# WestlyPark/StyleRenderer

Measured on AMD Instinct MI355X. Metric: generator fwd+bwd images/sec at 256^2, higher is better.
Workload: dtype f32

## Files before the change

### include/stylerenderer_amd.h

```cpp
#ifndef STYLERENDERER_AMD_H_
#define STYLERENDERER_AMD_H_

#include <stddef.h>
#include <stdint.h>

#ifdef __cplusplus
extern "C" {
#endif

typedef void* sr_stream_t;

#define SR_OK 0
#define SR_EINVAL (-1)
#define SR_ERANGE (-2)

const char* sr_error_string(int code);
int sr_abi_version(void);

int sr_fused_bias_act(float* y, const float* x, const float* b, const float* ref, int act, int grad,
                      float alpha, float scale, int64_t size_x, int64_t step_b, int64_t size_b,
                      int use_bias, int use_ref, sr_stream_t stream);

int64_t sr_fused_act_bwd_scratch_floats(int64_t n, int64_t c, int64_t inner);
int sr_fused_act_bwd(float* gx, float* gb, const float* gy, const float* out, float alpha,
// ... 34 lines not shown
int sr_adam_flat_guarded(float* p, const float* g, float* m, float* v, int64_t n, float lr, float beta1, float beta2,
                         float eps, float* step, const int64_t* guard_offs, int n_guards,
                         int32_t* skipped_host, sr_stream_t stream);

int64_t sr_rowdot_scratch_floats(int64_t rows, int64_t inner);
int sr_rowdot(float* dots, float* out_scaled, const float* a, const float* b, const float* scale,
              int64_t rows, int64_t inner, float* scratch, sr_stream_t stream);
int sr_rowdot_div(float* dots, const float* a, const float* b, const float* rdiv, int64_t rows, int64_t inner,
                  float* scratch, sr_stream_t stream);
int sr_rowdot_bwd(float* ga, float* gb, float* gs, const float* a, const float* b, const float* gd, const float* go,
                  const float* scale, int64_t rows, int64_t inner, float* scratch, sr_stream_t stream);

int sr_smallconv_fwd(float* out, const float* x, const float* ws, const float* bias, int64_t B, int64_t C,
                     int64_t N, int64_t hw, sr_stream_t stream);
int sr_smallconv_dx(float* dx, const float* g, const float* ws, int64_t B, int64_t C, int64_t N, int64_t hw,
                    sr_stream_t stream);
int sr_smallconv_dx_add(float* dx, const float* g, const float* ws, const float* addend, int64_t B, int64_t C, int64_t N,
                        int64_t hw, sr_stream_t stream);
int64_t sr_smallconv_dw_scratch_floats(int64_t B, int64_t C, int64_t N, int64_t hw);
int sr_smallconv_dw(float* dws, const float* g, const float* x, int64_t B, int64_t C, int64_t N, int64_t hw,
                    float* scratch, sr_stream_t stream);
int sr_smallconv_dw_bias(float* dws, float* gb, const float* g, const float* x, int64_t B, int64_t C, int64_t N, int64_t hw,
                         float* scratch, sr_stream_t stream);
int sr_modrows_fwd(float* ws, const float* w, const float* s, float scale, int64_t B, int64_t N, int64_t C,
                   sr_stream_t stream);
int sr_modrows_bwd(float* gs, float* gw, const float* dws, const float* w, const float* s, float scale, int64_t B,
                   int64_t N, int64_t C, sr_stream_t stream);

int sr_vertex_normals_f32(float* vn, float* norm_out, const float* v, const int64_t* tri, const int32_t* adj_off,
                          const int32_t* adj, int64_t B, int64_t nv, int64_t nf, float eps, sr_stream_t stream);

int sr_affine3_fwd(float* out, const float* v, const float* m, const float* t, int64_t B, int64_t nv,
                   int64_t v_bstride, sr_stream_t stream);
int sr_affine3_bwd(float* gm, float* gt, const float* v, const float* g, int64_t B, int64_t nv, int64_t v_bstride,
                   sr_stream_t stream);

int sr_morph_fwd(float* v, float* vs, float* reg, const float* w, const float* bias, const float* coeff, const float* lin,
                 const float* pose, const float* sigma, float lam, int64_t B, int64_t nv, int64_t d, sr_stream_t stream);
int sr_vertex_normals_bwd_f32(float* gvs, const float* gv, const float* gn, const float* lin, const float* rot,
                              const float* v, const float* ns, const float* normc, const int64_t* tri,
                              const int32_t* adj_off, const int32_t* adj, int64_t B, int64_t nv, int64_t nf, float eps,
                              sr_stream_t stream);
int64_t sr_morph_gcoeff_scratch_floats(int64_t rows, int64_t B, int64_t d);
int sr_morph_gcoeff(float* gcoeff, float* scratch, const float* w, const float* gvs, const float* coeff,
                    const float* sigma, float lam, const float* greg, int64_t B, int64_t rows, int64_t d,
                    sr_stream_t stream);
// ... 350 lines not shown
```

### stylerenderer_amd/_lib.py

```python
import ctypes
import os

_HERE = os.path.dirname(os.path.abspath(__file__))
LIB_PATH = os.environ.get("STYLERENDERER_AMD_LIB") or os.path.join(_HERE, "libstylerenderer_hip.so")

_i = ctypes.c_int
_l = ctypes.c_int64
_f = ctypes.c_float
_d = ctypes.c_double
_p = ctypes.c_void_p

SIGNATURES = {
    "sr_error_string": (ctypes.c_char_p, [_i]),
    "sr_abi_version": (_i, []),
    "sr_fused_bias_act": (_i, [_p, _p, _p, _p, _i, _i, _f, _f, _l, _l, _l, _i, _i, _p]),
    "sr_fused_act_bwd_scratch_floats": (_l, [_l, _l, _l]),
    "sr_fused_act_bwd": (_i, [_p, _p, _p, _p, _f, _f, _l, _l, _l, _p, _p]),
    "sr_noise_bias_act": (_i, [_p] * 6 + [_f, _f] + [_l] * 4 + [_p]),
    "sr_noise_bias_act_bwd_scratch_floats": (_l, [_l, _l, _l]),
    "sr_noise_bias_act_bwd": (_i, [_p] * 6 + [_f, _f] + [_l] * 4 + [_p, _p]),
    "sr_noise_bias_act_bwd_dot_scratch_floats": (_l, [_l, _l, _l]),
    "sr_noise_bias_act_bwd_dot": (_i, [_p] * 9 + [_f, _f] + [_l] * 4 + [_p, _p]),
    "sr_conv2d_nba": (_i, [_p] * 8 + [_f, _f] + [_l] * 7 + [_p, _p]),
    "sr_conv2d_nba_ex": (_i, [_p] * 8 + [_f, _f] + [_l] * 7 + [_i, _p, _p]),
    "sr_noise_bias_act_affine": (_i, [_p] * 4 + [_l] + [_p] * 3 + [_f, _f] + [_l] * 4 + [_p]),
    "sr_noise_bias_act_affine_bwd_scratch_floats": (_l, [_l, _l, _l]),
    "sr_noise_bias_act_affine_bwd": (_i, [_p] * 9 + [_l, _p, _f, _f] + [_l] * 4 + [_p, _p]),
    "sr_noise_bias_act_affine_bwd2_scratch_floats": (_l, [_l, _l, _l]),
    "sr_noise_bias_act_affine_bwd2": (_i, [_p, _p, _p, _l, _p, _p, _l] + [_p] * 6 + [_l, _p, _f, _f] + [_l] * 4 + [_p, _p]),
    "sr_adam_flat": (_i, [_p] * 4 + [_l] + [_f] * 4 + [_p, _p]),
    "sr_adam_flat_guarded": (_i, [_p] * 4 + [_l] + [_f] * 4 + [_p, ctypes.POINTER(_l), _i, _p, _p]),
    "sr_rowdot_scratch_floats": (_l, [_l, _l]),
    "sr_rowdot": (_i, [_p] * 5 + [_l, _l, _p, _p]),
    "sr_rowdot_div": (_i, [_p] * 4 + [_l, _l, _p, _p]),
    "sr_rowdot_bwd": (_i, [_p] * 8 + [_l, _l, _p, _p]),
    "sr_smallconv_fwd": (_i, [_p] * 4 + [_l] * 4 + [_p]),
    "sr_smallconv_dx": (_i, [_p] * 3 + [_l] * 4 + [_p]),
    "sr_smallconv_dx_add": (_i, [_p] * 4 + [_l] * 4 + [_p]),
    "sr_smallconv_dw_scratch_floats": (_l, [_l] * 4),
    "sr_smallconv_dw": (_i, [_p] * 3 + [_l] * 4 + [_p, _p]),
    "sr_smallconv_dw_bias": (_i, [_p] * 4 + [_l] * 4 + [_p, _p]),
    "sr_modrows_fwd": (_i, [_p] * 3 + [_f] + [_l] * 3 + [_p]),
    "sr_modrows_bwd": (_i, [_p] * 5 + [_f] + [_l] * 3 + [_p]),
    "sr_vertex_normals_f32": (_i, [_p] * 6 + [_l] * 3 + [_f, _p]),
    "sr_linear_fwd": (_i, [_p] * 4 + [_l] * 4 + [_f, _f, _i, _f, _f, _p]),
    "sr_linear_bwd_x": (_i, [_p] * 4 + [_l] * 3 + [_f, _i, _f, _f, _p]),
    "sr_linear_bwd_w": (_i, [_p] * 5 + [_l] * 4 + [_f, _f, _i, _f, _f, _p]),
    "sr_demod_fwd": (_i, [_p] * 3 + [_l] * 3 + [_f, _p]),
    "sr_demod_bwd": (_i, [_p] * 7 + [_l] * 3 + [_p]),
    "sr_weight_prep": (_i, [_p, _p, _p, _f, _l, _l, _i, _l, _p]),
    "sr_weight_prep_bwd": (_i, [_p, _p, _p, _p, _f, _l, _l, _i, _l, _p]),
    "sr_weight_adjoint": (_i, [_p, _p, _l, _l, _l, _l, _l, _i, _p]),
    "sr_bank_nt": (_i, [_i] + [_p] * 8 + [_l, _f, _f, _p]),
    "sr_bank_nn": (_i, [_i] + [_p] * 8 + [_l, _f, _p]),
    "sr_bank_tn": (_i, [_i] + [_p] * 8 + [_l, _f, _f, _p]),
    "sr_weight_prep_batch": (_i, [_i] + [_p] * 9),
    "sr_weight_adjoint_batch": (_i, [_i] + [_p] * 9),
    "sr_lpips_layer_scratch_floats": (_l, [_l, _l]),
    "sr_lpips_layer_fwd": (_i, [_p] * 4 + [_l] * 4 + [_f, _p, _p]),
    "sr_lpips_layer_bwd": (_i, [_p] * 5 + [_l] * 4 + [_f, _p]),
    "sr_ppl_endpoints": (_i, [_p, _p, _p, _l, _p, _l, _l, _i, _i, _f, _p]),
    "sr_ppl_prep": (_i, [_p] * 4 + [_l] * 9 + [_p]),
    "sr_lpips_pair_scratch_floats": (_l, [_l, _l, _p]),
    "sr_lpips_pair": (_i, [_p] * 5 + [_l, _l, _f, _p, _p]),
# ... 162 lines not shown
```

### stylerenderer_amd/csrc/fused_elem.hip

```cpp
#include "common.h"

namespace {

constexpr int EB = 256;
constexpr int ECHUNK = EB * 16;

__device__ __forceinline__ void block_sum2(float& a, float& b, float* lds8) {
    a = sr_wave_sum(a);
    b = sr_wave_sum(b);
    const int lane = threadIdx.x & 63, wave = threadIdx.x >> 6;
    if (lane == 0) { lds8[wave] = a; lds8[4 + wave] = b; }
    __syncthreads();
    if (threadIdx.x == 0) {
        a = (lds8[0] + lds8[1]) + (lds8[2] + lds8[3]);
        b = (lds8[4] + lds8[5]) + (lds8[6] + lds8[7]);
    }
}

template <bool REF>
__global__ __launch_bounds__(EB) void k_nba_fwd(float* __restrict__ y, const float* __restrict__ x,
                                                const float* __restrict__ noise,
                                                const float* __restrict__ noise_w,
                                                const float* __restrict__ bias,
                                                const float* __restrict__ ref, float alpha, float scale,
// ... 952 lines not shown
        const dim3 grid((unsigned)chunks, (unsigned)(B * C));
        switch (N) {
            case 1: hipLaunchKernelGGL((k_smallconv_dw<1, 1>), grid, dim3(256), 0, st, scratch, g, x, (int)C, hw, chunks, direct, gsum); break;
            case 2: hipLaunchKernelGGL((k_smallconv_dw<2, 1>), grid, dim3(256), 0, st, scratch, g, x, (int)C, hw, chunks, direct, gsum); break;
            case 3: hipLaunchKernelGGL((k_smallconv_dw<3, 1>), grid, dim3(256), 0, st, scratch, g, x, (int)C, hw, chunks, direct, gsum); break;
            default: hipLaunchKernelGGL((k_smallconv_dw<4, 1>), grid, dim3(256), 0, st, scratch, g, x, (int)C, hw, chunks, direct, gsum); break;
        }
    }
    if (chunks > 1)
        hipLaunchKernelGGL(k_smallconv_dw_finish, dim3((unsigned)(B * C)), dim3(64), 0, st, dws, scratch, (int)C,
                           (int)N, chunks, B * C);
    if (gb)
        hipLaunchKernelGGL(k_smallconv_gb_finish, dim3(1), dim3(64), 0, st, gb, gsum, (int)N, (int)(B * chunks));
    return sr_launch_status();
}

extern "C" int sr_smallconv_dw(float* dws, const float* g, const float* x, int64_t B, int64_t C, int64_t N,
                               int64_t hw, float* scratch, sr_stream_t stream) {
    return sr_smallconv_dw_bias(dws, nullptr, g, x, B, C, N, hw, scratch, stream);
}

namespace {

__global__ __launch_bounds__(256) void k_modrows_fwd(float* __restrict__ ws, const float* __restrict__ w,
                                                     const float* __restrict__ s, float scale, int B, int N, int C) {
    const int64_t i = (int64_t)blockIdx.x * 256 + threadIdx.x;
    if (i >= (int64_t)B * N * C) return;
    const int c = (int)(i % C);
    const int j = (int)((i / C) % N);
    const int b = (int)(i / ((int64_t)C * N));
    ws[i] = (w[(int64_t)j * C + c] * scale) * s[(int64_t)b * C + c];
}

__global__ __launch_bounds__(256) void k_modrows_bwd(float* __restrict__ gs, float* __restrict__ gw,
                                                     const float* __restrict__ dws, const float* __restrict__ w,
                                                     const float* __restrict__ s, float scale, int B, int N, int C) {
    const int c = blockIdx.x * 256 + threadIdx.x;
    if (c >= C) return;
    const int r = blockIdx.y;
    if (r < B) {
        if (!gs) return;
        float acc = 0.0f;
        for (int j = 0; j < N; ++j) acc += dws[((int64_t)r * N + j) * C + c] * (w[(int64_t)j * C + c] * scale);
        gs[(int64_t)r * C + c] = acc;
    } else {
        if (!gw) return;
// ... 122 lines not shown
```

### stylerenderer_amd/layers.py

```python
import math
import os

import torch
from torch import nn
from torch.nn import functional as F

from .op import FusedLeakyReLU, fused_leaky_relu, upfirdn2d
from .op import conv as _conv
from .op import conv_generic as _convg
from .op import smallconv as _smallconv
from .op import style as _style
from .op.style_bank import StylePack
from .op.upfirdn2d import skip_down as _skip_down
from .op.weight_prep import weight_prep as _weight_prep
from .op.weight_prep import weight_prep_cached as _weight_prep_cached
from .op._dispatch import strict_native as _strict_native


def _fused_tails():
    import os

    return os.environ.get("SR_FUSED_TAILS", "1") != "0"


def make_kernel(k):
    k = torch.tensor(k, dtype=torch.float32)
    if k.dim() == 1:
        k = k[None, :] * k[:, None]
    return k / k.sum()


class PixelNorm(nn.Module):
# ... 219 lines not shown
            return _conv.conv2d(input, wt, s, d, None, "c3")
        return _conv.conv2d(input, wt, s, d, None, "c1")

    def _forward_generic(self, input, s, skip_blur=False):
        w = self.weight[0] * self.scale
        x = input * s[:, :, None, None]
        d = None
        if self.demodulate:
            wsq = w.pow(2).sum((2, 3)).t().contiguous()
            if _style.demod_supported(s, wsq):
                d = _style.demod_scale(s, wsq, self.eps)
            else:
                d = torch.rsqrt(((s * s)[:, :, None] * wsq[None]).sum(1) + self.eps)
        if self.upsample:
            out = _convg.conv_transpose2d_generic(x, w.transpose(0, 1), stride=2, padding=0)
        elif self.downsample:
            out = _convg.conv2d_generic(self.blur(x), w, None, 2, 0)
        else:
            out = _convg.conv2d_generic(x, w, None, 1, self.padding)
        if d is not None:
            out = out * d[:, :, None, None]
        return self.blur(out) if (self.upsample and not skip_blur) else out

    def forward_noise_bias_act(self, input, style, noise, noise_weight, act_bias, negative_slope, act_scale):
        if (input.device.type != "cuda" or self.upsample or self.downsample or self.kernel_size != 3
                or not self.demodulate or act_bias is None or not _fused_tails()):
            return None
        input = input.contiguous()
        if not _conv.conv_nba_shape_ok(input, self.out_channel, noise):
            return None
        s = self.style_of(style)
        if isinstance(style, StylePack) and style.d is not None:
            wt, wsq, d = style.wt, style.wsq, style.d
            if not _conv.conv_nba_supported(input, wt, noise):
                return None
        else:
            wt, wsq = self._wprep(True)
            if not (_conv.conv_nba_supported(input, wt, noise) and _style.demod_supported(s, wsq)):
                return None
            d = _style.demod_scale(s, wsq, self.eps)
        return _conv.conv2d_nba(input, wt, s, d, noise, noise_weight, act_bias, negative_slope, act_scale)

    def forward_up_noise_bias_act(self, input, style, noise, noise_weight, act_bias, negative_slope, act_scale):
        if (input.device.type != "cuda" or not self.upsample or self.kernel_size != 3 or not self.demodulate
                or act_bias is None or not _fused_tails()):
            return None
        s = self.style_of(style)
        pad = self.blur.pad
        oh = 2 * input.shape[2] + 1 + pad[0] + pad[1] - 3
        ow = 2 * input.shape[3] + 1 + pad[0] + pad[1] - 3
        if isinstance(style, StylePack) and style.d is not None:
            wt, wsq, d = style.wt, style.wsq, style.d
            if not _conv.upconv_nba_supported(input, wt, noise, oh, ow):
                return None
        else:
            wt, wsq = self._wprep(True)
            if not (_conv.upconv_nba_supported(input, wt, noise, oh, ow) and _style.demod_supported(s, wsq)):
                return None
            d = _style.demod_scale(s, wsq, self.eps)
        kernel = self.blur.kernel
        return _conv.upconv_nba(input.contiguous(), wt, s, d, kernel, pad, noise, noise_weight, act_bias,
                                negative_slope, act_scale)

# ... 202 lines not shown
```

### stylerenderer_amd/model.py

```python
import math

import numpy as np
import torch
from torch import nn

from .layers import (BiasBank, Blur, ConstantInput, ConvLayer, EqualLinear, ModulatedConv2d, NoiseInjection,
                     PixelNorm, ResBlock, Upsample)
from .op import FusedLeakyReLU, rasterize
from .op import smallconv as _smallconv
from .op import style_bank as _style_bank
from .op import weight_bank as _weight_bank
from .op.fused_elem import blur_noise_bias_act, noise_bias_act, noise_bias_act_affine
from .op.rasterize import rasterize_pyramid
from .op.upfirdn2d import upsample2_add

CHANNEL_BASE = {4: 512, 8: 512, 16: 512, 32: 512, 64: 256, 128: 128, 256: 64, 512: 32, 1024: 16}


def channel_table(channel_multiplier):
    return {r: (c if r <= 32 else c * channel_multiplier) for r, c in CHANNEL_BASE.items()}


class StyledConv(nn.Module):

    def __init__(self, in_channel, out_channel, kernel_size, style_dim, upsample=False,
                 blur_kernel=[1, 3, 3, 1], demodulate=True):
        super().__init__()
        self.conv = ModulatedConv2d(in_channel, out_channel, kernel_size, style_dim,
                                    upsample=upsample, blur_kernel=blur_kernel, demodulate=demodulate)
        self.noise = NoiseInjection()
        self.bias = None
        self.activate = FusedLeakyReLU(out_channel)

    def forward(self, input, style, noise=None):
        if noise is not None and noise.requires_grad:
            return self.activate(self.noise(self.conv(input, style), noise=noise))
        if input.device.type == "cuda" and self.conv.upsample:
            blur = self.conv.blur
            oh = 2 * input.shape[2] + 1 + sum(blur.pad) - 3
            ow = 2 * input.shape[3] + 1 + sum(blur.pad) - 3
            if noise is None:
                noise = input.new_empty(input.shape[0], 1, oh, ow).normal_()
            noise = noise.contiguous()
            fused = self.conv.forward_up_noise_bias_act(input, style, noise, self.noise.weight, self.activate.bias,
                                                        self.activate.negative_slope, self.activate.scale)
            if fused is not None:
                return fused
            y = self.conv(input, style, skip_blur=True)
            return blur_noise_bias_act(y, blur.kernel, blur.pad, noise, self.noise.weight, self.activate.bias,
                                       self.activate.negative_slope, self.activate.scale)
        if input.device.type == "cuda":
            if noise is None:
                noise = input.new_empty(input.shape[0], 1, input.shape[2], input.shape[3]).normal_()
            fused = self.conv.forward_noise_bias_act(input, style, noise.contiguous(), self.noise.weight,
                                                     self.activate.bias, self.activate.negative_slope,
                                                     self.activate.scale)
            if fused is not None:
                return fused
            out = self.conv(input, style)
            return noise_bias_act(out, noise, self.noise.weight, self.activate.bias,
                                  self.activate.negative_slope, self.activate.scale)
        out = self.conv(input, style)
        out = self.noise(out, noise=noise)
        return self.activate(out)


class StyledMapConv(nn.Module):

    def __init__(self, in_channel, out_channel, kernel_size, style_dim, upsample=False,
                 blur_kernel=[1, 3, 3, 1], demodulate=True):
        super().__init__()
        self.conv = ModulatedConv2d(in_channel, out_channel, kernel_size, style_dim,
                                    upsample=upsample, blur_kernel=blur_kernel, demodulate=demodulate)
        self.noise = NoiseInjection()
        self.bias = None
        self.activate = FusedLeakyReLU(out_channel)

    def forward(self, input, style, stylemap, noise=None):
        out = self.conv(input, style)
# ... 17 lines not shown
class ToRGB(nn.Module):
    def __init__(self, in_channel, style_dim, upsample=True, blur_kernel=[1, 3, 3, 1]):
        super().__init__()
        if upsample:
            self.upsample = Upsample(blur_kernel)
        self.conv = ModulatedConv2d(in_channel, 3, 1, style_dim, demodulate=False)
        self.bias = nn.Parameter(torch.zeros(1, 3, 1, 1))

    def forward(self, input, style, skip=None, fork=False):
        conv = self.conv
        if _smallconv.supported(input, conv.out_channel):
            out = _smallconv.modulated_conv1x1_small(input, conv.weight.view(conv.out_channel, conv.in_channel),
                                                     conv.style_of(style), self.bias.view(-1), scale=conv.scale,
                                                     fork=fork and _fork_enabled())
            if fork and _fork_enabled():
                input, out = out
            if skip is not None:
                out = upsample2_add(skip, self.upsample.kernel, self.upsample.pad, out)
            return (input, out) if fork else out
        out = self.conv(input, style) + self.bias
        if skip is not None:
            out = out + self.upsample(skip)
        return (input, out) if fork else out


class Generator(nn.Module):
    def __init__(self, size, style_dim, n_mlp, channel_multiplier=2, blur_kernel=[1, 3, 3, 1],
                 lr_mlp=0.01):
        super().__init__()
        self._build_trunk(size, style_dim, n_mlp, channel_multiplier, lr_mlp)
        self._build_synthesis(StyledConv, style_dim, blur_kernel)

    def _build_trunk(self, size, style_dim, n_mlp, channel_multiplier, lr_mlp):
        self.size = size
        self.style_dim = style_dim
        mapping = [PixelNorm()]
        mapping += [EqualLinear(style_dim, style_dim, lr_mul=lr_mlp, activation="fused_lrelu")
                    for _ in range(n_mlp)]
        self.style = nn.Sequential(*mapping)
        self.channels = channel_table(channel_multiplier)
        self.input = ConstantInput(self.channels[4])
        self.to_rgb1 = ToRGB(self.channels[4], style_dim, upsample=False)
        self.log_size = int(math.log(size, 2))
        self.num_layers = (self.log_size - 2) * 2 + 1
        self.n_latent = self.log_size * 2 - 2
        self.convs = nn.ModuleList()
# ... 92 lines not shown
            i += 2
        return seq

    def _layer_styles(self, latent):
        seq = self._style_layers()
        if latent.device.type == "cuda" and latent.dtype == torch.float32 and _style_bank.enabled():
            return _style_bank.build(seq, latent)
        rows = latent.unbind(1)
        return [rows[li] for _, li in seq]

    def forward(self, styles, return_latents=False, inject_index=None, truncation=1,
                truncation_latent=None, input_is_latent=False, noise=None, randomize_noise=True):
        latent, noise = self._latents(styles, inject_index, truncation, truncation_latent,
                                      input_is_latent, noise, randomize_noise)
        with _weight_bank.Scope(self):
            out = self.input(latent)
            st = self._layer_styles(latent)
            out = self.conv1(out, st[0], noise=noise[0])
            out, skip = self.to_rgb1(out, st[1], fork=True)
            k = 2
            for conv_up, conv, n_up, n_conv, to_rgb in zip(self.convs[::2], self.convs[1::2],
                                                           noise[1::2], noise[2::2], self.to_rgbs):
                out = conv_up(out, st[k], noise=n_up)
                out = conv(out, st[k + 1], noise=n_conv)
                out, skip = to_rgb(out, st[k + 2], skip, fork=True)
                k += 3
        return skip, (latent if return_latents else None)


class GeneratorWithMap(Generator):
    def __init__(self, size, style_dim, n_mlp, n_stylemap=3, channel_multiplier=2,
                 blur_kernel=[1, 3, 3, 1], lr_mlp=0.01):
        nn.Module.__init__(self)
        self._build_trunk(size, style_dim, n_mlp, channel_multiplier, lr_mlp)
        self.norm_to_style = nn.ModuleList()
        if n_stylemap != 3:
            self.norm1 = nn.Sequential(ConvLayer(3, n_stylemap, 3), ResBlock(n_stylemap, 2, downsample=False))
        else:
            self.norm1 = ResBlock(n_stylemap, 2, downsample=False)

        def add_map_heads():
            if n_stylemap != 3:
                self.norm_to_style.append(ConvLayer(3, n_stylemap, 3))
            self.norm_to_style.append(ResBlock(n_stylemap, 4, downsample=False))

        self._build_synthesis(StyledMapConv, style_dim, blur_kernel, per_resolution=add_map_heads)

    def forward(self, styles, mesh, return_normals=False, return_latents=False, inject_index=None,
# ... 8 lines not shown
    def _synthesis_with_maps(self, latent, noise, vert, attr, tri, return_normals, return_latents):
        out = self.input(latent)
        res0 = (int(out.shape[2]), int(out.shape[3]))
        pyramid = _normal_pyramid(vert, attr, tri, [(res0[0] << k, res0[1] << k)
                                                     for k in range(min(len(self.convs) // 2, len(self.to_rgbs)) + 1)])
        norm_maps = [pyramid[0] if pyramid else _normal_map(vert, attr, tri, res0[0], res0[1])]
        maps = self.norm1(norm_maps[-1].contiguous())
        st = self._layer_styles(latent)
        out = self.conv1(out, st[0], maps, noise=noise[0])
        out, skip = self.to_rgb1(out, st[1], fork=True)
        two_stage = len(self.convs) == len(self.norm_to_style)
        i, k = 1, 2
        for conv_up, conv, n_up, n_conv, to_rgb in zip(self.convs[::2], self.convs[1::2],
                                                       noise[1::2], noise[2::2], self.to_rgbs):
            norm_maps.append(pyramid[len(norm_maps)] if pyramid else
                             _normal_map(vert, attr, tri, 2 * int(out.shape[2]), 2 * int(out.shape[3])))
            nm = norm_maps[-1].contiguous()
            if two_stage:
                maps = self.norm_to_style[i](self.norm_to_style[i - 1](nm))
            else:
                maps = self.norm_to_style[i // 2](nm)
            maps_up, maps_conv = maps.split([2, maps.shape[1] - 2], 1)
            out = conv_up(out, st[k], maps_up, noise=n_up)
            out = conv(out, st[k + 1], maps_conv, noise=n_conv)
            out, skip = to_rgb(out, st[k + 2], skip, fork=True)
            i += 2
            k += 3
        return skip, (latent if return_latents else None), (norm_maps if return_normals else None)


def _normal_pyramid(vert, attr, tri, sizes):
    import os

    if (vert.device.type != "cuda" or vert.dim() != 3 or attr.dim() != 3 or os.environ.get("SR_RASTER_NCHW", "1") == "0"
            or os.environ.get("SR_RASTER_PYRAMID", "1") == "0"):
        return None
    return rasterize_pyramid(vert, attr, tri, sizes, channel_major=True)


def _normal_map(vert, attr, tri, h, w):
    import os

    if os.environ.get("SR_RASTER_NCHW", "1") != "0":
        return rasterize(vert, attr, tri, h, w, channel_major=True)
    return rasterize(vert, attr, tri, h, w).permute(0, 3, 1, 2)


class Discriminator(nn.Module):
# ... 32 lines not shown
```

### stylerenderer_amd/op/conv.py

```python
import os
import threading

import torch

from .. import _lib
from ._dispatch import hold_for_capture, mark_inputs, native, require_f32, wanted
from . import weight_prep as _wp
from . import wgrad_style as _ws
from .fused_elem import noise_stride, param_grads, rowdot, rowdot_div


PROFILE = None


def _timed(like, kind, geom, flops, launch):
    if PROFILE is None:
        return launch()
    stream = torch.cuda.current_stream(like.device)
    e0, e1 = torch.cuda.Event(enable_timing=True), torch.cuda.Event(enable_timing=True)
    e0.record(stream)
    launch()
    e1.record(stream)
    PROFILE.append((kind, geom, flops, e0, e1))

# ... 244 lines not shown
    if x.device.type != "cuda" or x.dtype != torch.float32 or not x.is_contiguous():
        return False
    b, c, h, w = x.shape
    ok = b * n <= 65535 and _lib.lib().sr_conv2d_path(b, c, n, h, w, h, w, 3, 1, 1, 0, _lib.ptr(x), None, None, 0,
                                                      1) == _lib.CONV_PATH_WINO
    if noise is not None:
        ok = ok and noise.dtype == torch.float32 and noise.numel() in (h * w, b * h * w) and noise.data_ptr() % 16 == 0
    return ok


def conv_nba_supported(x, wt, noise):
    return wt.shape[0] == 9 and conv_nba_shape_ok(x, wt.shape[2], noise)


def _wt_pitch(wt):
    taps, cw, n = wt.shape
    if (wt.stride(2) == 1 and wt.stride(1) % 4 == 0 and wt.stride(1) >= n and wt.stride(0) == cw * wt.stride(1)
            and wt.data_ptr() % 16 == 0):
        return wt, wt.stride(1)
    ldw = (n + 3) // 4 * 4
    return (torch.nn.functional.pad(wt, (0, ldw - n)) if ldw != n else wt.contiguous()), ldw


class ConvNBAFn(torch.autograd.Function):
    @staticmethod
    def forward(ctx, x, wt, iscale, oscale, noise, noise_w, abias, slope, gain):
        mark_inputs(ctx, x, wt, iscale, oscale, noise, noise_w, abias, slope, gain)
        b, c, h, w = x.shape
        n = wt.shape[2]
        wtp, ldw = _wt_pitch(wt)
        out = torch.empty((b, n, h, w), dtype=x.dtype, device=x.device)
        nscr = _lib.lib().sr_conv2d_scratch_floats(b, c, n, h, w, h, w, 3, 1, 1, 0)
        scratch, flags, entry = _conv_scratch(wt if wtp is wt else wtp, max(nscr, 1), (b, c, n, h, w, 3, 1, 1, False), x)
        flops = 2.0 * b * h * w * c * n * 9
        _timed(x, "conv", (3, 1, 0, b, c, n, h, w), flops,
               lambda: native(x).sr_conv2d_nba_ex(out, x, wtp, iscale, oscale, noise, noise_w, abias, float(slope),
                                                  float(gain), b, c, n, ldw, h, w, noise_stride(noise, h * w), flags,
                                                  scratch))
        _scratch_written(entry, b, c, n, h, w, x, out)
        ctx.save_for_backward(x, wt, iscale, oscale, noise, noise_w, abias, out)
        ctx.cfg = (float(slope), float(gain))
        ctx.frozen = bool(getattr(wt, "_sr_frozen", False))
        ctx.adj = getattr(wt, "_sr_adj", None)
        return out

    @staticmethod
    def backward(ctx, gy):
        from .fused_elem import _NBA

        x, wt, iscale, oscale, noise, noise_w, abias, out = ctx.saved_tensors
        slope, gain = ctx.cfg
        needs = wanted(ctx)
        if torch.is_grad_enabled() and oscale is not None:
            return _recorded_backward(
                (x, wt, iscale, oscale, None, noise_w, abias), needs, gy,
                lambda xa, wa, sa, da, _, nwa, aba: _NBA.apply(ConvFn.apply(xa, wa, sa, da, None, "c3"), noise, nwa, aba,
                                                               slope, gain, out.detach()))
        want_p = bool(needs[6] or (noise is not None and needs[5]))
        if oscale is None:
            from .fused_elem import _NBABackward

            g, gb, gnw = _NBABackward.apply(gy, out, noise, slope, gain, want_p)
            rdot = None
        else:
            g, gb, gnw, rdot = _nba_bwd_dot(gy, out, noise, noise_w, abias, slope, gain, want_p)
        gos = None
        gx, gw, gis = _conv_grads(x, g, wt, iscale, oscale, "c3", needs[0], needs[1], needs[2], ctx.frozen, ctx.adj)
        if needs[3] and oscale is not None:
            gos = rdot / oscale
        return (gx, gw, gis, gos, None, (gnw if noise is not None and want_p and needs[5] else None),
                (gb if want_p and needs[6] else None), None, None)


def _nba_bwd_dot(gy, out, noise, noise_w, abias, slope, gain, want_params=True):
    gy = gy.contiguous()
    b, n, h, w = out.shape
    inner = h * w
    g = torch.empty_like(out)
    gb, gnw = param_grads(out, noise, want_params)
    rdot = torch.empty((b, n), dtype=out.dtype, device=out.device)
    scratch = torch.empty(_lib.lib().sr_noise_bias_act_bwd_dot_scratch_floats(b, n, inner), dtype=out.dtype,
                          device=out.device)
    native(out).sr_noise_bias_act_bwd_dot(g, gb, gnw, rdot, gy, out, noise, noise_w, abias, slope, gain, b, n, inner,
                                          noise_stride(noise, inner), scratch)
    return g, gb, gnw, rdot


def _blur_bwd_fused():
    import os

    return os.environ.get("SR_BLUR_BWD_FUSED", "1") != "0"


def _blur_nba_bwd(gy, out, k_flipped, p0, shape257, noise, noise_w, abias, slope, gain, want_params=True):
# ... 127 lines not shown
```

### stylerenderer_amd/op/smallconv.py

```python
import torch
from torch.autograd import Function

from .. import _lib
from ._dispatch import mark_inputs, native, wanted


def supported(x, n_out):
    return (x.device.type == "cuda" and x.dtype == torch.float32 and x.dim() == 4 and 1 <= n_out <= 4
            and (x.size(2) * x.size(3)) % 4 == 0 and x.size(0) * x.size(1) <= 65535 and x.size(1) <= 4096)


def _aligned(t):
    t = t.contiguous()
    return t if t.data_ptr() % 16 == 0 else t.clone()


def _fwd(x, ws, bias=None):
    x, ws = _aligned(x), ws.contiguous()
    b, c, h, w = x.shape
    n = ws.size(1)
    out = torch.empty((b, n, h, w), dtype=x.dtype, device=x.device)
    native(x).sr_smallconv_fwd(out, x, ws, bias.contiguous() if bias is not None else None, b, c, n, h * w)
    return out

# ... 33 lines not shown
        want_b = len(needs) > 2 and needs[2]
        gw = gb = None
        if needs[1] and want_b:
            gw, gb = SmallConvDwBias.apply(g, x)
        elif needs[1]:
            gw = SmallConvDw.apply(g, x)
        elif want_b:
            gb = g.sum((0, 2, 3))
        return gx, gw, gb


class SmallConvFork(Function):

    @staticmethod
    def forward(ctx, x, ws, bias=None):
        mark_inputs(ctx, x, ws, bias)
        ctx.save_for_backward(x, ws)
        ctx.set_materialize_grads(False)
        return x.view_as(x), _fwd(x, ws, bias)

    @staticmethod
    def backward(ctx, g_x, g):
        x, ws = ctx.saved_tensors
        needs = wanted(ctx)
        if g is None:
            return (g_x if needs[0] else None), None, None
        gx = None
        if needs[0]:
            fused = (g_x is not None and not torch.is_grad_enabled() and g_x.is_contiguous() and g_x.data_ptr() % 16 == 0
                     and g_x.dtype == g.dtype and g_x.shape == x.shape)
            if fused:
                gx = _dx(g, ws, g_x)
            else:
                gx = SmallConvDx.apply(g, ws)
                if g_x is not None:
                    gx = gx + g_x
        want_b = len(needs) > 2 and needs[2]
        gw = gb = None
        if needs[1] and want_b:
            gw, gb = SmallConvDwBias.apply(g, x)
        elif needs[1]:
            gw = SmallConvDw.apply(g, x)
        elif want_b:
            gb = g.sum((0, 2, 3))
        return gx, gw, gb


class SmallConvDx(Function):
    @staticmethod
    def forward(ctx, g, ws):
        ctx.save_for_backward(g, ws)
        return _dx(g, ws)

    @staticmethod
    def backward(ctx, gg):
        g, ws = ctx.saved_tensors
        d_g = SmallConvFwd.apply(gg, ws) if ctx.needs_input_grad[0] else None
        d_ws = SmallConvDw.apply(g, gg) if ctx.needs_input_grad[1] else None
        return d_g, d_ws


class SmallConvDw(Function):
    @staticmethod
    def forward(ctx, g, x):
        ctx.save_for_backward(g, x)
        return _dw(g, x)

    @staticmethod
# ... 79 lines not shown
```

Measured before the change: 610.6.

## Fuse conv noise-bias-act backward with toRGB 1x1 conv backward in one kernel

Adds a combined autograd function for the styled conv plus its toRGB 1x1 head, with a single HIP kernel for the backward pass. That kernel computes the toRGB dx, the leaky-ReLU gradient, the bias and noise-weight partial sums, the demod row-dot, the 1x1 weight gradient and the RGB bias sum in one read of the activations. This removes several separate elementwise and reduction kernels and the intermediate gradient tensor traffic between them. The cost is a more complex kernel with many accumulators per thread, which raises register pressure, and it needs extra finish launches when the spatial size spans more than one chunk.

```diff
diff --git a/include/stylerenderer_amd.h b/include/stylerenderer_amd.h
--- a/include/stylerenderer_amd.h
+++ b/include/stylerenderer_amd.h
@@ -80,6 +80,11 @@
                     float* scratch, sr_stream_t stream);
 int sr_smallconv_dw_bias(float* dws, float* gb, const float* g, const float* x, int64_t B, int64_t C, int64_t N, int64_t hw,
                          float* scratch, sr_stream_t stream);
+int64_t sr_fork_nba_bwd_scratch_floats(int64_t B, int64_t C, int64_t N, int64_t hw);
+int sr_fork_nba_bwd(float* gpre, float* gbias, float* gnoise_w, float* rowdot, float* dws, float* gb_rgb,
+                    const float* g_above, const float* y, const float* g_rgb, const float* ws, const float* noise,
+                    const float* noise_w, const float* bias, float alpha, float scale, int64_t B, int64_t C, int64_t N,
+                    int64_t hw, int64_t noise_bstride, float* scratch, sr_stream_t stream);
 int sr_modrows_fwd(float* ws, const float* w, const float* s, float scale, int64_t B, int64_t N, int64_t C,
                    sr_stream_t stream);
 int sr_modrows_bwd(float* gs, float* gw, const float* dws, const float* w, const float* s, float scale, int64_t B,
diff --git a/stylerenderer_amd/_lib.py b/stylerenderer_amd/_lib.py
--- a/stylerenderer_amd/_lib.py
+++ b/stylerenderer_amd/_lib.py
@@ -40,6 +40,8 @@
     "sr_smallconv_dw_scratch_floats": (_l, [_l] * 4),
     "sr_smallconv_dw": (_i, [_p] * 3 + [_l] * 4 + [_p, _p]),
     "sr_smallconv_dw_bias": (_i, [_p] * 4 + [_l] * 4 + [_p, _p]),
+    "sr_fork_nba_bwd_scratch_floats": (_l, [_l] * 4),
+    "sr_fork_nba_bwd": (_i, [_p] * 13 + [_f, _f] + [_l] * 5 + [_p, _p]),
     "sr_modrows_fwd": (_i, [_p] * 3 + [_f] + [_l] * 3 + [_p]),
     "sr_modrows_bwd": (_i, [_p] * 5 + [_f] + [_l] * 3 + [_p]),
     "sr_vertex_normals_f32": (_i, [_p] * 6 + [_l] * 3 + [_f, _p]),
diff --git a/stylerenderer_amd/csrc/fused_elem.hip b/stylerenderer_amd/csrc/fused_elem.hip
--- a/stylerenderer_amd/csrc/fused_elem.hip
+++ b/stylerenderer_amd/csrc/fused_elem.hip
@@ -998,6 +998,190 @@
 
 namespace {
 
+template <int N, int CH>
+__global__ __launch_bounds__(EB) void k_fork_nba_bwd(float* __restrict__ gpre, float* __restrict__ partial,
+                                                     float* __restrict__ dot_partial, float* __restrict__ dw_partial,
+                                                     float* __restrict__ dws, float* __restrict__ gsum,
+                                                     const float* __restrict__ addend, const float* __restrict__ y,
+                                                     const float* __restrict__ g, const float* __restrict__ ws,
+                                                     const float* __restrict__ noise, const float* __restrict__ noise_w,
+                                                     const float* __restrict__ bias, float alpha, float scale,
+                                                     float inv_pos, float inv_neg, int C, int64_t hw,
+                                                     int64_t noise_bstride, int chunks) {
+    __shared__ float lds_nba[CH][2][8];
+    __shared__ float lds[CH][4 * SC_MAXN];
+    __shared__ float lds_g[4 * SC_MAXN];
+    const int64_t row0 = (int64_t)blockIdx.y * CH;
+    const int64_t b = row0 / C;
+    const int c0 = (int)(row0 - b * C);
+    const int64_t off = (int64_t)blockIdx.x * ECHUNK;
+    const int64_t remain = hw - off;
+    const int n4 = (int)((remain < ECHUNK ? remain : ECHUNK) / 4);
+    const float4* ns = noise ? reinterpret_cast<const float4*>(noise + b * noise_bstride + off) : nullptr;
+    const float nw = noise ? noise_w[0] : 0.0f;
+    float w[CH][N], bb[CH];
+#pragma unroll
+    for (int k = 0; k < CH; ++k) {
+        bb[k] = bias ? bias[c0 + k] : 0.0f;
+#pragma unroll
+        for (int j = 0; j < N; ++j) w[k][j] = ws[(b * N + j) * C + c0 + k];
+    }
+    float acc[CH][N], sb[CH], sn[CH], sd[CH], ag[N];
+#pragma unroll
+    for (int k = 0; k < CH; ++k) {
+        sb[k] = sn[k] = sd[k] = 0.0f;
+#pragma unroll
+        for (int j = 0; j < N; ++j) acc[k][j] = 0.0f;
+    }
+#pragma unroll
+    for (int j = 0; j < N; ++j) ag[j] = 0.0f;
+    const bool sum_g = gsum != nullptr && c0 == 0;
+    for (int i = threadIdx.x; i < n4; i += EB) {
+        float4 gg[N], a[CH], o[CH];
+#pragma unroll
+        for (int j = 0; j < N; ++j) gg[j] = reinterpret_cast<const float4*>(g + (b * N + j) * hw + off)[i];
+#pragma unroll
+        for (int k = 0; k < CH; ++k) {
+            o[k] = reinterpret_cast<const float4*>(y + (row0 + k) * hw + off)[i];
+            if (addend) a[k] = reinterpret_cast<const float4*>(addend + (row0 + k) * hw + off)[i];
+        }
+        float4 nz = make_float4(0.f, 0.f, 0.f, 0.f);
+        if (noise) nz = ns[i];
+        if (sum_g) {
+#pragma unroll
+            for (int j = 0; j < N; ++j) ag[j] += (gg[j].x + gg[j].y) + (gg[j].z + gg[j].w);
+        }
+#pragma unroll
+        for (int k = 0; k < CH; ++k) {
+            float4 gy = make_float4(0.f, 0.f, 0.f, 0.f);
+#pragma unroll
+            for (int j = 0; j < N; ++j) {
+                gy.x += w[k][j] * gg[j].x; gy.y += w[k][j] * gg[j].y; gy.z += w[k][j] * gg[j].z; gy.w += w[k][j] * gg[j].w;
+            }
+            if (addend) { gy.x = a[k].x + gy.x; gy.y = a[k].y + gy.y; gy.z = a[k].z + gy.z; gy.w = a[k].w + gy.w; }
+            const float4 v = o[k];
+            float4 r;
+            r.x = ((v.x > 0.0f) ? gy.x : gy.x * alpha) * scale;
+            r.y = ((v.y > 0.0f) ? gy.y : gy.y * alpha) * scale;
+            r.z = ((v.z > 0.0f) ? gy.z : gy.z * alpha) * scale;
+            r.w = ((v.w > 0.0f) ? gy.w : gy.w * alpha) * scale;
+            reinterpret_cast<float4*>(gpre + (row0 + k) * hw + off)[i] = r;
+            sb[k] += (r.x + r.y) + (r.z + r.w);
+            if (noise) sn[k] += (r.x * nz.x + r.y * nz.y) + (r.z * nz.z + r.w * nz.w);
+            const float y0 = ((v.x > 0.0f) ? v.x * inv_pos : v.x * inv_neg) - nw * nz.x - bb[k];
+            const float y1 = ((v.y > 0.0f) ? v.y * inv_pos : v.y * inv_neg) - nw * nz.y - bb[k];
+            const float y2 = ((v.z > 0.0f) ? v.z * inv_pos : v.z * inv_neg) - nw * nz.z - bb[k];
+            const float y3 = ((v.w > 0.0f) ? v.w * inv_pos : v.w * inv_neg) - nw * nz.w - bb[k];
+            sd[k] += (r.x * y0 + r.y * y1) + (r.z * y2 + r.w * y3);
+#pragma unroll
+            for (int j = 0; j < N; ++j)
+                acc[k][j] += (v.x * gg[j].x + v.y * gg[j].y) + (v.z * gg[j].z + v.w * gg[j].w);
+        }
+    }
+#pragma unroll
+    for (int k = 0; k < CH; ++k) {
+        float dummy = 0.0f;
+        block_sum2(sb[k], sn[k], lds_nba[k][0]);
+        block_sum2(sd[k], dummy, lds_nba[k][1]);
+    }
+    if (threadIdx.x == 0) {
+#pragma unroll
+        for (int k = 0; k < CH; ++k) {
+            partial[((row0 + k) * chunks + blockIdx.x) * 2] = sb[k];
+            partial[((row0 + k) * chunks + blockIdx.x) * 2 + 1] = sn[k];
+            dot_partial[(row0 + k) * chunks + blockIdx.x] = sd[k];
+        }
+    }
+    const int lane = threadIdx.x & 63, wave = threadIdx.x >> 6;
+#pragma unroll
+    for (int k = 0; k < CH; ++k)
+#pragma unroll
+        for (int j = 0; j < N; ++j) {
+            const float r = sr_wave_sum(acc[k][j]);
+            if (lane == 0) lds[k][j * 4 + wave] = r;
+        }
+    if (sum_g) {
+#pragma unroll
+        for (int j = 0; j < N; ++j) {
+            const float r = sr_wave_sum(ag[j]);
+            if (lane == 0) lds_g[j * 4 + wave] = r;
+        }
+    }
+    __syncthreads();
+    if (sum_g && threadIdx.x >= 64 && threadIdx.x < 64 + N) {
+        const int j = threadIdx.x - 64;
+        gsum[(b * chunks + blockIdx.x) * N + j] = (lds_g[j * 4] + lds_g[j * 4 + 1]) + (lds_g[j * 4 + 2] + lds_g[j * 4 + 3]);
+    }
+    if (threadIdx.x < CH * N) {
+        const int k = threadIdx.x / N, j = threadIdx.x % N;
+        const float r = (lds[k][j * 4] + lds[k][j * 4 + 1]) + (lds[k][j * 4 + 2] + lds[k][j * 4 + 3]);
+        if (dws) dws[(b * N + j) * C + (c0 + k)] = r;
+        else dw_partial[((row0 + k) * chunks + blockIdx.x) * N + j] = r;
+    }
+}
+
+constexpr int FORK_CH = 4;
+
+inline int64_t fork_nba_floats(int64_t B, int64_t C, int64_t hw) {
+    const int64_t n = 3 * B * C * sr_ceil_div(hw, ECHUNK) + C + 2;
+    return n + (n & 1);
+}
+
+}
+
+extern "C" int64_t sr_fork_nba_bwd_scratch_floats(int64_t B, int64_t C, int64_t N, int64_t hw) {
+    if (B <= 0 || C <= 0 || N <= 0 || hw <= 0) return 4;
+    return fork_nba_floats(B, C, hw) + B * C * sr_ceil_div(hw, ECHUNK) * N + B * sr_ceil_div(hw, ECHUNK) * N + 1;
+}
+
+extern "C" int sr_fork_nba_bwd(float* gpre, float* gbias, float* gnoise_w, float* rowdot, float* dws, float* gb_rgb,
+                               const float* g_above, const float* y, const float* g_rgb, const float* ws,
+                               const float* noise, const float* noise_w, const float* bias, float alpha, float scale,
+                               int64_t B, int64_t C, int64_t N, int64_t hw, int64_t noise_bstride, float* scratch,
+                               sr_stream_t stream) {
+    if (!gpre || !rowdot || !dws || !y || !g_rgb || !ws || !scratch || (noise && !noise_w) || scale == 0.0f ||
+        alpha == 0.0f)
+        return SR_EINVAL;
+    if (!smallconv_ok(B, C, N, hw, g_rgb, y) || hw <= 0 || C % FORK_CH != 0 || B * C > 65535) return SR_EINVAL;
+    if (!vec_ok(hw, gpre, g_above, y, noise) || (noise && noise_bstride % 4 != 0) || gpre == g_above) return SR_EINVAL;
+    const int chunks = (int)sr_ceil_div(hw, ECHUNK);
+    hipStream_t st = sr_stream(stream);
+    const int64_t rows = B * C;
+    float* dot_scratch = scratch + 2 * rows * chunks;
+    float* chan_nw = dot_scratch + rows * chunks;
+    float* dw_scratch = scratch + fork_nba_floats(B, C, hw);
+    float* dot_partial = chunks == 1 ? rowdot : dot_scratch;
+    float* direct = chunks == 1 ? dws : nullptr;
+    float* gsum = gb_rgb ? dw_scratch + rows * chunks * N : nullptr;
+    const dim3 grid((unsigned)chunks, (unsigned)(rows / FORK_CH));
+#define SR_FORK_NBA(NN)                                                                                                    \
+    hipLaunchKernelGGL((k_fork_nba_bwd<NN, FORK_CH>), grid, dim3(EB), 0, st, gpre, scratch, dot_partial, dw_scratch, direct,  \
+                       gsum, g_above, y, g_rgb, ws, noise, noise_w, bias, alpha, scale, 1.0f / scale,                       \
+                       1.0f / (alpha * scale), (int)C, hw, noise_bstride, chunks)
+    switch (N) {
+        case 1: SR_FORK_NBA(1); break;
+        case 2: SR_FORK_NBA(2); break;
+        case 3: SR_FORK_NBA(3); break;
+        default: SR_FORK_NBA(4); break;
+    }
+#undef SR_FORK_NBA
+    if (gbias) {
+        hipLaunchKernelGGL(k_nba_finish, dim3((unsigned)C), dim3(64), 0, st, gbias, chan_nw, scratch, B, (int)C, chunks);
+        if (noise && gnoise_w)
+            hipLaunchKernelGGL(k_nba_finish2, dim3(1), dim3(64), 0, st, gnoise_w, chan_nw, (int)C);
+    }
+    if (chunks > 1) {
+        hipLaunchKernelGGL(k_rowdot_finish, dim3((unsigned)rows), dim3(64), 0, st, rowdot, dot_partial, chunks);
+        hipLaunchKernelGGL(k_smallconv_dw_finish, dim3((unsigned)rows), dim3(64), 0, st, dws, dw_scratch, (int)C, (int)N,
+                           chunks, rows);
+    }
+    if (gb_rgb)
+        hipLaunchKernelGGL(k_smallconv_gb_finish, dim3(1), dim3(64), 0, st, gb_rgb, gsum, (int)N, (int)(B * chunks));
+    return sr_launch_status();
+}
+
+namespace {
+
 __global__ __launch_bounds__(256) void k_modrows_fwd(float* __restrict__ ws, const float* __restrict__ w,
                                                      const float* __restrict__ s, float scale, int B, int N, int C) {
     const int64_t i = (int64_t)blockIdx.x * 256 + threadIdx.x;
diff --git a/stylerenderer_amd/layers.py b/stylerenderer_amd/layers.py
--- a/stylerenderer_amd/layers.py
+++ b/stylerenderer_amd/layers.py
@@ -8,6 +8,7 @@
 from .op import FusedLeakyReLU, fused_leaky_relu, upfirdn2d
 from .op import conv as _conv
 from .op import conv_generic as _convg
+from .op import fork_tail as _fork_tail
 from .op import smallconv as _smallconv
 from .op import style as _style
 from .op.style_bank import StylePack
@@ -273,7 +274,7 @@
             out = out * d[:, :, None, None]
         return self.blur(out) if (self.upsample and not skip_blur) else out
 
-    def forward_noise_bias_act(self, input, style, noise, noise_weight, act_bias, negative_slope, act_scale):
+    def forward_noise_bias_act(self, input, style, noise, noise_weight, act_bias, negative_slope, act_scale, fork=None):
         if (input.device.type != "cuda" or self.upsample or self.downsample or self.kernel_size != 3
                 or not self.demodulate or act_bias is None or not _fused_tails()):
             return None
@@ -290,6 +291,12 @@
             if not (_conv.conv_nba_supported(input, wt, noise) and _style.demod_supported(s, wsq)):
                 return None
             d = _style.demod_scale(s, wsq, self.eps)
+        if fork is not None and _fork_tail.enabled():
+            if _fork_tail.supported(input, self.out_channel, fork.n_rgb, noise, d):
+                ws, rgb_bias = fork.rows()
+                out, fork.rgb = _fork_tail.conv2d_nba_fork(input, wt, s, d, noise, noise_weight, act_bias, negative_slope,
+                                                           act_scale, ws, rgb_bias)
+                return out
         return _conv.conv2d_nba(input, wt, s, d, noise, noise_weight, act_bias, negative_slope, act_scale)
 
     def forward_up_noise_bias_act(self, input, style, noise, noise_weight, act_bias, negative_slope, act_scale):
diff --git a/stylerenderer_amd/model.py b/stylerenderer_amd/model.py
--- a/stylerenderer_amd/model.py
+++ b/stylerenderer_amd/model.py
@@ -7,6 +7,7 @@
 from .layers import (BiasBank, Blur, ConstantInput, ConvLayer, EqualLinear, ModulatedConv2d, NoiseInjection,
                      PixelNorm, ResBlock, Upsample)
 from .op import FusedLeakyReLU, rasterize
+from .op import fork_tail as _fork_tail
 from .op import smallconv as _smallconv
 from .op import style_bank as _style_bank
 from .op import weight_bank as _weight_bank
@@ -32,7 +33,7 @@
         self.bias = None
         self.activate = FusedLeakyReLU(out_channel)
 
-    def forward(self, input, style, noise=None):
+    def forward(self, input, style, noise=None, fork=None):
         if noise is not None and noise.requires_grad:
             return self.activate(self.noise(self.conv(input, style), noise=noise))
         if input.device.type == "cuda" and self.conv.upsample:
@@ -54,7 +55,7 @@
                 noise = input.new_empty(input.shape[0], 1, input.shape[2], input.shape[3]).normal_()
             fused = self.conv.forward_noise_bias_act(input, style, noise.contiguous(), self.noise.weight,
                                                      self.activate.bias, self.activate.negative_slope,
-                                                     self.activate.scale)
+                                                     self.activate.scale, fork=fork)
             if fused is not None:
                 return fused
             out = self.conv(input, style)
@@ -118,6 +119,26 @@
         if skip is not None:
             out = out + self.upsample(skip)
         return (input, out) if fork else out
+
+    def fork_head(self, style):
+        conv = self.conv
+        return _fork_tail.Head(conv.out_channel, lambda: (
+            _smallconv.modulated_rows(conv.weight.view(conv.out_channel, conv.in_channel), conv.style_of(style), conv.scale),
+            self.bias.view(-1)))
+
+
+def _conv_to_rgb(conv, to_rgb, out, s_conv, s_rgb, skip, noise, *maps):
+    if not maps and isinstance(conv, StyledConv) and _fork_enabled() and _fork_tail.enabled():
+        head = to_rgb.fork_head(s_rgb)
+        out = conv(out, s_conv, noise=noise, fork=head)
+        if head.rgb is not None:
+            rgb = head.rgb
+            if skip is not None:
+                rgb = upsample2_add(skip, to_rgb.upsample.kernel, to_rgb.upsample.pad, rgb)
+            return out, rgb
+    else:
+        out = conv(out, s_conv, *maps, noise=noise)
+    return to_rgb(out, s_rgb, skip, fork=True)
 
 
 class Generator(nn.Module):
@@ -256,8 +277,7 @@
             for conv_up, conv, n_up, n_conv, to_rgb in zip(self.convs[::2], self.convs[1::2],
                                                            noise[1::2], noise[2::2], self.to_rgbs):
                 out = conv_up(out, st[k], noise=n_up)
-                out = conv(out, st[k + 1], noise=n_conv)
-                out, skip = to_rgb(out, st[k + 2], skip, fork=True)
+                out, skip = _conv_to_rgb(conv, to_rgb, out, st[k + 1], st[k + 2], skip, n_conv)
                 k += 3
         return skip, (latent if return_latents else None)
 
@@ -312,8 +332,7 @@
                 maps = self.norm_to_style[i // 2](nm)
             maps_up, maps_conv = maps.split([2, maps.shape[1] - 2], 1)
             out = conv_up(out, st[k], maps_up, noise=n_up)
-            out = conv(out, st[k + 1], maps_conv, noise=n_conv)
-            out, skip = to_rgb(out, st[k + 2], skip, fork=True)
+            out, skip = _conv_to_rgb(conv, to_rgb, out, st[k + 1], st[k + 2], skip, n_conv, maps_conv)
             i += 2
             k += 3
         return skip, (latent if return_latents else None), (norm_maps if return_normals else None)
diff --git a/stylerenderer_amd/op/conv.py b/stylerenderer_amd/op/conv.py
--- a/stylerenderer_amd/op/conv.py
+++ b/stylerenderer_amd/op/conv.py
@@ -290,22 +290,58 @@
     return (torch.nn.functional.pad(wt, (0, ldw - n)) if ldw != n else wt.contiguous()), ldw
 
 
+def _nba_forward(x, wt, iscale, oscale, noise, noise_w, abias, slope, gain):
+    b, c, h, w = x.shape
+    n = wt.shape[2]
+    wtp, ldw = _wt_pitch(wt)
+    out = torch.empty((b, n, h, w), dtype=x.dtype, device=x.device)
+    nscr = _lib.lib().sr_conv2d_scratch_floats(b, c, n, h, w, h, w, 3, 1, 1, 0)
+    scratch, flags, entry = _conv_scratch(wt if wtp is wt else wtp, max(nscr, 1), (b, c, n, h, w, 3, 1, 1, False), x)
+    flops = 2.0 * b * h * w * c * n * 9
+    _timed(x, "conv", (3, 1, 0, b, c, n, h, w), flops,
+           lambda: native(x).sr_conv2d_nba_ex(out, x, wtp, iscale, oscale, noise, noise_w, abias, float(slope),
+                                              float(gain), b, c, n, ldw, h, w, noise_stride(noise, h * w), flags,
+                                              scratch))
+    _scratch_written(entry, b, c, n, h, w, x, out)
+    return out
+
+
+def _nba_backward(saved, cfg, frozen, adj, needs, gy):
+    from .fused_elem import _NBA
+
+    x, wt, iscale, oscale, noise, noise_w, abias, out = saved
+    slope, gain = cfg
+    if torch.is_grad_enabled() and oscale is not None:
+        return _recorded_backward(
+            (x, wt, iscale, oscale, None, noise_w, abias), needs, gy,
+            lambda xa, wa, sa, da, _, nwa, aba: _NBA.apply(ConvFn.apply(xa, wa, sa, da, None, "c3"), noise, nwa, aba,
+                                                           slope, gain, out.detach()))
+    want_p = bool(needs[6] or (noise is not None and needs[5]))
+    if oscale is None:
+        from .fused_elem import _NBABackward
+
+        g, gb, gnw = _NBABackward.apply(gy, out, noise, slope, gain, want_p)
+        rdot = None
+    else:
+        g, gb, gnw, rdot = _nba_bwd_dot(gy, out, noise, noise_w, abias, slope, gain, want_p)
+    return _nba_grads(saved, frozen, adj, needs, want_p, g, gb, gnw, rdot)
+
+
+def _nba_grads(saved, frozen, adj, needs, want_p, g, gb, gnw, rdot):
+    x, wt, iscale, oscale, noise = saved[:5]
+    gos = None
+    gx, gw, gis = _conv_grads(x, g, wt, iscale, oscale, "c3", needs[0], needs[1], needs[2], frozen, adj)
+    if needs[3] and oscale is not None:
+        gos = rdot / oscale
+    return (gx, gw, gis, gos, None, (gnw if noise is not None and want_p and needs[5] else None),
+            (gb if want_p and needs[6] else None), None, None)
+
+
 class ConvNBAFn(torch.autograd.Function):
     @staticmethod
     def forward(ctx, x, wt, iscale, oscale, noise, noise_w, abias, slope, gain):
         mark_inputs(ctx, x, wt, iscale, oscale, noise, noise_w, abias, slope, gain)
-        b, c, h, w = x.shape
-        n = wt.shape[2]
-        wtp, ldw = _wt_pitch(wt)
-        out = torch.empty((b, n, h, w), dtype=x.dtype, device=x.device)
-        nscr = _lib.lib().sr_conv2d_scratch_floats(b, c, n, h, w, h, w, 3, 1, 1, 0)
-        scratch, flags, entry = _conv_scratch(wt if wtp is wt else wtp, max(nscr, 1), (b, c, n, h, w, 3, 1, 1, False), x)
-        flops = 2.0 * b * h * w * c * n * 9
-        _timed(x, "conv", (3, 1, 0, b, c, n, h, w), flops,
-               lambda: native(x).sr_conv2d_nba_ex(out, x, wtp, iscale, oscale, noise, noise_w, abias, float(slope),
-                                                  float(gain), b, c, n, ldw, h, w, noise_stride(noise, h * w), flags,
-                                                  scratch))
-        _scratch_written(entry, b, c, n, h, w, x, out)
+        out = _nba_forward(x, wt, iscale, oscale, noise, noise_w, abias, slope, gain)
         ctx.save_for_backward(x, wt, iscale, oscale, noise, noise_w, abias, out)
         ctx.cfg = (float(slope), float(gain))
         ctx.frozen = bool(getattr(wt, "_sr_frozen", False))
@@ -314,30 +350,7 @@
 
     @staticmethod
     def backward(ctx, gy):
-        from .fused_elem import _NBA
-
-        x, wt, iscale, oscale, noise, noise_w, abias, out = ctx.saved_tensors
-        slope, gain = ctx.cfg
-        needs = wanted(ctx)
-        if torch.is_grad_enabled() and oscale is not None:
-            return _recorded_backward(
-                (x, wt, iscale, oscale, None, noise_w, abias), needs, gy,
-                lambda xa, wa, sa, da, _, nwa, aba: _NBA.apply(ConvFn.apply(xa, wa, sa, da, None, "c3"), noise, nwa, aba,
-                                                               slope, gain, out.detach()))
-        want_p = bool(needs[6] or (noise is not None and needs[5]))
-        if oscale is None:
-            from .fused_elem import _NBABackward
-
-            g, gb, gnw = _NBABackward.apply(gy, out, noise, slope, gain, want_p)
-            rdot = None
-        else:
-            g, gb, gnw, rdot = _nba_bwd_dot(gy, out, noise, noise_w, abias, slope, gain, want_p)
-        gos = None
-        gx, gw, gis = _conv_grads(x, g, wt, iscale, oscale, "c3", needs[0], needs[1], needs[2], ctx.frozen, ctx.adj)
-        if needs[3] and oscale is not None:
-            gos = rdot / oscale
-        return (gx, gw, gis, gos, None, (gnw if noise is not None and want_p and needs[5] else None),
-                (gb if want_p and needs[6] else None), None, None)
+        return _nba_backward(ctx.saved_tensors, ctx.cfg, ctx.frozen, ctx.adj, wanted(ctx), gy)
 
 
 def _nba_bwd_dot(gy, out, noise, noise_w, abias, slope, gain, want_params=True):
diff --git a/stylerenderer_amd/op/fork_tail.py b/stylerenderer_amd/op/fork_tail.py
--- /dev/null
+++ b/stylerenderer_amd/op/fork_tail.py
@@ -0,0 +1,81 @@
+import os
+
+import torch
+
+from .. import _lib
+from . import conv as _conv
+from . import smallconv as _smallconv
+from ._dispatch import mark_inputs, native, wanted
+from .fused_elem import noise_stride, param_grads
+
+
+def enabled():
+    return os.environ.get("SR_FORK_TAIL", "1") != "0"
+
+
+class Head:
+    __slots__ = ("n_rgb", "rows", "rgb")
+
+    def __init__(self, n_rgb, rows):
+        self.n_rgb, self.rows, self.rgb = n_rgb, rows, None
+
+
+def supported(x, n, n_rgb, noise, oscale):
+    b, _, h, w = x.shape
+    return (oscale is not None and 1 <= n_rgb <= 4 and n % 4 == 0 and n <= 4096
+            and (h * w) % 4 == 0 and b * n <= 65535)
+
+
+def _fused_backward(g_y, g_rgb, out, ws, noise, noise_w, abias, slope, gain, want_params, want_rgb_bias):
+    g_rgb, ws = _smallconv._aligned(g_rgb), ws.contiguous()
+    b, n, h, w = out.shape
+    nrgb = ws.size(1)
+    inner = h * w
+    gpre = torch.empty_like(out)
+    gb, gnw = param_grads(out, noise, want_params)
+    rdot = torch.empty((b, n), dtype=out.dtype, device=out.device)
+    dws = torch.empty((b, nrgb, n), dtype=out.dtype, device=out.device)
+    gb_rgb = torch.empty(nrgb, dtype=out.dtype, device=out.device) if want_rgb_bias else None
+    scratch = torch.empty(_lib.lib().sr_fork_nba_bwd_scratch_floats(b, n, nrgb, inner), dtype=out.dtype, device=out.device)
+    native(out).sr_fork_nba_bwd(gpre, gb, gnw, rdot, dws, gb_rgb, g_y, out, g_rgb, ws, noise, noise_w, abias, slope, gain,
+                                b, n, nrgb, inner, noise_stride(noise, inner), scratch)
+    return gpre, gb, gnw, rdot, dws, gb_rgb
+
+
+class ConvNBAForkFn(torch.autograd.Function):
+    @staticmethod
+    def forward(ctx, x, wt, iscale, oscale, noise, noise_w, abias, slope, gain, ws, rgb_bias):
+        mark_inputs(ctx, x, wt, iscale, oscale, noise, noise_w, abias, slope, gain, ws, rgb_bias)
+        out = _conv._nba_forward(x, wt, iscale, oscale, noise, noise_w, abias, slope, gain)
+        rgb = _smallconv._fwd(out, ws, rgb_bias)
+        ctx.save_for_backward(x, wt, iscale, oscale, noise, noise_w, abias, out, ws)
+        ctx.cfg = (float(slope), float(gain))
+        ctx.frozen = bool(getattr(wt, "_sr_frozen", False))
+        ctx.adj = getattr(wt, "_sr_adj", None)
+        ctx.set_materialize_grads(False)
+        return out, rgb
+
+    @staticmethod
+    def backward(ctx, g_y, g_rgb):
+        saved, ws = ctx.saved_tensors[:8], ctx.saved_tensors[8]
+        noise, noise_w, abias, out = saved[4:]
+        slope, gain = ctx.cfg
+        needs = wanted(ctx)
+        if g_y is None and g_rgb is None:
+            return (None,) * 11
+        fused = (g_rgb is not None and not torch.is_grad_enabled() and needs[9] and slope != 0.0 and gain != 0.0
+                 and out.data_ptr() % 16 == 0
+                 and (g_y is None or (g_y.is_contiguous() and g_y.data_ptr() % 16 == 0 and g_y.dtype == out.dtype
+                                      and g_y.shape == out.shape)))
+        if not fused:
+            gy, gws, gb_rgb = _smallconv.fork_backward(out, ws, (True, needs[9], needs[10]), g_y, g_rgb)
+            return _conv._nba_backward(saved, ctx.cfg, ctx.frozen, ctx.adj, needs[:9], gy) + (gws, gb_rgb)
+        want_p = bool(needs[6] or (noise is not None and needs[5]))
+        gpre, gb, gnw, rdot, dws, gb_rgb = _fused_backward(g_y, g_rgb, out, ws, noise, noise_w, abias, slope, gain, want_p,
+                                                           needs[10])
+        return _conv._nba_grads(saved, ctx.frozen, ctx.adj, needs[:9], want_p, gpre, gb, gnw, rdot) + (dws, gb_rgb)
+
+
+def conv2d_nba_fork(x, wt, iscale, oscale, noise, noise_w, abias, slope, gain, ws, rgb_bias):
+    y, rgb = ConvNBAForkFn.apply(x, wt, iscale, oscale, noise, noise_w, abias, slope, gain, ws, rgb_bias)
+    return y.view_as(y), rgb
diff --git a/stylerenderer_amd/op/smallconv.py b/stylerenderer_amd/op/smallconv.py
--- a/stylerenderer_amd/op/smallconv.py
+++ b/stylerenderer_amd/op/smallconv.py
@@ -79,28 +79,31 @@
     @staticmethod
     def backward(ctx, g_x, g):
         x, ws = ctx.saved_tensors
-        needs = wanted(ctx)
-        if g is None:
-            return (g_x if needs[0] else None), None, None
-        gx = None
-        if needs[0]:
-            fused = (g_x is not None and not torch.is_grad_enabled() and g_x.is_contiguous() and g_x.data_ptr() % 16 == 0
-                     and g_x.dtype == g.dtype and g_x.shape == x.shape)
-            if fused:
-                gx = _dx(g, ws, g_x)
-            else:
-                gx = SmallConvDx.apply(g, ws)
-                if g_x is not None:
-                    gx = gx + g_x
-        want_b = len(needs) > 2 and needs[2]
-        gw = gb = None
-        if needs[1] and want_b:
-            gw, gb = SmallConvDwBias.apply(g, x)
-        elif needs[1]:
-            gw = SmallConvDw.apply(g, x)
-        elif want_b:
-            gb = g.sum((0, 2, 3))
-        return gx, gw, gb
+        return fork_backward(x, ws, wanted(ctx), g_x, g)
+
+
+def fork_backward(x, ws, needs, g_x, g):
+    if g is None:
+        return (g_x if needs[0] else None), None, None
+    gx = None
+    if needs[0]:
+        fused = (g_x is not None and not torch.is_grad_enabled() and g_x.is_contiguous() and g_x.data_ptr() % 16 == 0
+                 and g_x.dtype == g.dtype and g_x.shape == x.shape)
+        if fused:
+            gx = _dx(g, ws, g_x)
+        else:
+            gx = SmallConvDx.apply(g, ws)
+            if g_x is not None:
+                gx = gx + g_x
+    want_b = len(needs) > 2 and needs[2]
+    gw = gb = None
+    if needs[1] and want_b:
+        gw, gb = SmallConvDwBias.apply(g, x)
+    elif needs[1]:
+        gw = SmallConvDw.apply(g, x)
+    elif want_b:
+        gb = g.sum((0, 2, 3))
+    return gx, gw, gb
 
 
 class SmallConvDx(Function):
```

After: 624.1 (median of 6 runs). 1.02x the previous value.
